# ada-shen/Interpret_quality

Measured on AMD Instinct MI355X. Metric: coalitions/sec (masked forward passes/sec), PointNet 1024-pt ModelNet10, higher is better.
Workload: dtype f32; 1 GPU; PointNet ModelNet10-style Shapley, 32 regions x 1000 permutations per cloud (33000 coalitions per step per GPU), BASELINE configs[1]; permutations sampled and masked on the device inside the timed step; num_points=1024, num_regions=32, permutations=1000, parallelism=clouds sharded over 1 GPU(s), one all_gather_into_tensor of the logits per step

## Files before the change

interpret_quality_amd/csrc/iq_api.hip:

```cpp
#include <algorithm>
#include <vector>

#include "../../include/iq_debug.h"
#include "iq_common.h"
#include "iq_profile.h"

extern "C" int iq_version(void) { return IQ_ABI_VERSION; }

extern "C" const char* iq_last_error(void) { return iq::err_buf(); }

namespace iq {
namespace {
struct Span { hipEvent_t start, stop; int which; double work; };
struct ThreadState {
    std::vector<Span> spans;
    bool enabled = false;
    bool no_lds_gemm = false;
    int twin = 0;
};
ThreadState& ts() {
    static thread_local ThreadState s;
    return s;
}
}

bool profile_enabled() { return ts().enabled; }

bool no_lds_gemm() { return ts().no_lds_gemm; }
int twin() { return ts().twin; }

ProfileSpan::ProfileSpan(int which, hipStream_t st, double work) : which_(which), st_(st), on_(ts().enabled), work_(work) {
    if (!on_) return;
    (void)hipEventCreate(&start_);
    (void)hipEventCreate(&stop_);
    (void)hipEventRecord(start_, st_);
}

ProfileSpan::~ProfileSpan() {
    if (!on_) return;
    (void)hipEventRecord(stop_, st_);
    ts().spans.push_back(Span{start_, stop_, which_, work_});
}
}

extern "C" int iq_set_tuning(int key, int value) {
    if (key == iq::kTuneNoLdsGemm && (value == 0 || value == 1)) {
        iq::ts().no_lds_gemm = value != 0;
        return IQ_OK;
    }
    if (key == iq::kTuneTwin) {
        switch (value) {
            case 0: case iq::kTwinEdgeGemmL2: case iq::kTwinEdgeGemmLds: case iq::kTwinKnnCompact: case iq::kTwinPcKnn:
            case iq::kTwinPcGroupedMlp: case iq::kTwinKnnFp32Rank: case iq::kTwinPn2MemberWalk: case iq::kTwinKnnFp32Mfma:
            case iq::kTwinPcTwoKernel: case iq::kTwinChainL3Fp32: case iq::kTwinChainL3Fp32NoTail16: case iq::kTwinGroupFp32:
            case iq::kTwinDenseFp32: case iq::kTwinChainL3Single: case iq::kTwinDenseTile128: case iq::kTwinGroupFp32Chunk64:
                iq::ts().twin = value;
                return IQ_OK;
        }
    }
    return iq::fail(IQ_EINVAL, "iq_set_tuning: key %d value %d is not an experiment knob", key, value);
}

extern "C" int iq_profile_enable(int on) {
    iq::ts().enabled = on != 0;
    return IQ_OK;
}

extern "C" int iq_profile_read_work(int which, double* total_ms, int* launches, double* total_work) {
    IQ_REQUIRE(total_ms && launches, "iq_profile_read: null output");
    double tot = 0.0, work = 0.0;
    int n = 0;
    std::vector<iq::Span> rest;
    for (const iq::Span& s : iq::ts().spans) {
        if (s.which != which) { rest.push_back(s); continue; }
        float ms = 0.f;
        if (hipEventSynchronize(s.stop) != hipSuccess || hipEventElapsedTime(&ms, s.start, s.stop) != hipSuccess)
            return iq::fail(IQ_ELAUNCH, "iq_profile_read: event query failed");
        tot += ms;
        work += s.work;
        ++n;
        (void)hipEventDestroy(s.start);
        (void)hipEventDestroy(s.stop);
    }
    iq::ts().spans.swap(rest);
    *total_ms = tot;
    *launches = n;
    if (total_work) *total_work = work;
    return IQ_OK;
}

extern "C" int iq_profile_read(int which, double* total_ms, int* launches) {
    return iq_profile_read_work(which, total_ms, launches, nullptr);
}

namespace {
typedef float dbg_f32x16 __attribute__((ext_vector_type(16)));
typedef __bf16 dbg_bf16x8 __attribute__((ext_vector_type(8)));
typedef unsigned dbg_u32x4 __attribute__((ext_vector_type(4)));
__device__ unsigned long long g_sustained_clk[2];

__device__ inline dbg_bf16x8 dbg_operand(unsigned seed) {
    dbg_u32x4 v;
    for (int i = 0; i < 4; ++i) {
        seed = seed * 1664525u + 1013904223u;
        const unsigned lo = 0x3f80u | ((seed >> 9) & 0x7fu) | ((seed >> 3) & 0x8000u);
        seed = seed * 1664525u + 1013904223u;
        const unsigned hi = 0x3f80u | ((seed >> 9) & 0x7fu) | ((seed >> 3) & 0x8000u);
        v[i] = lo | (hi << 16);
    }
    return __builtin_bit_cast(dbg_bf16x8, v);
}

__global__ __launch_bounds__(256) void mfma_sustained_kernel(float* out, int iters, int seed0) {
    const dbg_bf16x8 a0 = dbg_operand(seed0 + threadIdx.x * 7 + blockIdx.x), a1 = dbg_operand(seed0 * 3 + threadIdx.x * 11 + blockIdx.x);
    const dbg_bf16x8 b0 = dbg_operand(seed0 * 5 + threadIdx.x * 13), b1 = dbg_operand(seed0 * 9 + threadIdx.x * 17);
    unsigned long long t0 = 0, r0 = 0;
    if (threadIdx.x == 0 && blockIdx.x == 0) {
        asm volatile("s_memtime %0\n\ts_waitcnt lgkmcnt(0)" : "=s"(t0)::"memory");
        r0 = __builtin_amdgcn_s_memrealtime();
    }
    dbg_f32x16 c0 = {0}, c1 = {0}, c2 = {0}, c3 = {0};
    for (int it = 0; it < iters; ++it) {
#pragma unroll
        for (int r = 0; r < 4; ++r) {
            c0 = __builtin_amdgcn_mfma_f32_32x32x16_bf16(a0, b0, c0, 0, 0, 0);
            c1 = __builtin_amdgcn_mfma_f32_32x32x16_bf16(a1, b0, c1, 0, 0, 0);
            c2 = __builtin_amdgcn_mfma_f32_32x32x16_bf16(a0, b1, c2, 0, 0, 0);
            c3 = __builtin_amdgcn_mfma_f32_32x32x16_bf16(a1, b1, c3, 0, 0, 0);
        }
    }
    if (threadIdx.x == 0 && blockIdx.x == 0) {
        unsigned long long t1;
        asm volatile("s_memtime %0\n\ts_waitcnt lgkmcnt(0)" : "=s"(t1)::"memory");
        g_sustained_clk[0] = t1 - t0;
        g_sustained_clk[1] = __builtin_amdgcn_s_memrealtime() - r0;
    }
    out[blockIdx.x * blockDim.x + threadIdx.x] = c0[0] + c1[5] + c2[9] + c3[15];
}
// ... 76 lines not shown
```

interpret_quality_amd/csrc/iq_common.h:

```cpp
#pragma once
#include <hip/hip_runtime.h>

#include <cstdarg>
#include <cstdio>

#include "../../include/iq.h"

namespace iq {

inline char* err_buf() {
    static thread_local char buf[512] = {0};
    return buf;
}

inline int fail(int code, const char* fmt, ...) {
    va_list ap;
    va_start(ap, fmt);
    vsnprintf(err_buf(), 512, fmt, ap);
    va_end(ap);
    return code;
}

inline int check_launch(const char* what) {
    hipError_t e = hipGetLastError();
    if (e != hipSuccess) return fail(IQ_ELAUNCH, "%s: %s", what, hipGetErrorString(e));
    return IQ_OK;
}

inline hipStream_t as_stream(iq_stream_t s) { return reinterpret_cast<hipStream_t>(s); }

inline size_t align_up(size_t x, size_t a) { return (x + a - 1) / a * a; }

__host__ __device__ inline bool keep_bit(unsigned long long keep, int rid) {
    return (unsigned)rid < 64u && ((keep >> rid) & 1ull);
}

constexpr int kMaxKeepWords = IQ_MAX_WIDE_REGIONS / 64;

__host__ __device__ inline int keep_words(int R) { return (R + 63) >> 6; }

__device__ __forceinline__ bool keep_bit_wide(const uint64_t* keep, int rid, int R) {
    return (unsigned)rid < (unsigned)R && ((keep[rid >> 6] >> (rid & 63)) & 1ull);
}

template <bool WIDE>
struct WaveKeep {
    unsigned long long k = 0;
    const uint64_t* row = nullptr;
    int R = 64;
    __device__ __forceinline__ WaveKeep(const uint64_t* keep, int b, int R_, int W, int lane, uint64_t* strip) {
        if constexpr (WIDE) {
            if (lane < W) strip[lane] = keep[(size_t)b * W + lane];
            __builtin_amdgcn_fence(__ATOMIC_RELEASE, "wavefront");
            __builtin_amdgcn_wave_barrier();
            __builtin_amdgcn_fence(__ATOMIC_ACQUIRE, "wavefront");
            row = strip;
            R = R_;
        } else {
            k = keep[b];
        }
    }
    __device__ __forceinline__ bool operator()(int rid) const {
        if constexpr (WIDE) return keep_bit_wide(row, rid, R);
        else return keep_bit(k, rid);
    }
};

__device__ inline int xcd_cloud(int block, int wgs_per_cloud, int B) {
    const int c = ((block >> 3) / wgs_per_cloud) * 8 + (block & 7);
    return (c | 3) < B ? (c & ~3) | ((c + (c >> 3)) & 3) : c;
}

}

#define IQ_REQUIRE(cond, ...) \
    do {                      \
        if (!(cond)) return iq::fail(IQ_EINVAL, __VA_ARGS__); \
    } while (0)
```

interpret_quality_amd/csrc/iq_pointnet.hip:

```cpp
#include <algorithm>
#include <type_traits>

#include "iq_common.h"
#include "iq_profile.h"

#include "iq_bf3.h"
#include "iq_mfma.h"

namespace {

constexpr int kFeat = IQ_NUM_FEAT;
constexpr int kMC = 64;
constexpr int kMC96 = 96;
constexpr int kMaxN = 4096;
constexpr int kThreads = 256;
constexpr int kRowCap = kMaxN + kMC;

enum ChainMode { kPrepool = 0, kFstn = 1, kTrunk = 2, kFstn64 = 3, kTrunk64 = 4 };

constexpr int kLd1 = 64 + 4;
constexpr int kLd2 = 128 + 4;

struct ChainArgs {
    const float* clouds;
    int ps, cs, cl;
    const float* centers;
    const uint16_t* rows;
    const int32_t* nrows;
    const int32_t* item_order;
    const int32_t* cloud_of;
    const float* trans;
    const float* w_in;
    const float* w1;
    const float* b1;
    const float* w2;
    const float* b2;
    const float* w3;
    const float* b3;
    const unsigned short* w3_bf3;
    const unsigned short* w2_bf3;
    float* out;
    int32_t* argrow;
    int N, R, items, nclouds, with_centre;
    int tail16;
    int l3_single;
};

struct BRing {
    f32x4 r[8];
};

__device__ __forceinline__ void bring_init(BRing& ring, const WBuf& w3, int wave_s) {
#pragma unroll
    for (int i = 0; i < 8; ++i) ring.r[i] = wbuf_load(w3, (wave_s * 16 + i) * kFragBytes);
}

template <int MTS, bool ARGMAX = false>
__device__ __forceinline__ void l3_pass_v2(const WBuf& w3, const float* abase, int wave_s, float (&runmax)[8], BRing& ring,
                                           int (&runarg)[8], int rowbase = 0, int fh = 0) {
    const int w0 = wave_s * 16 * kFragBytes;
    int wq = w0;
#pragma unroll 1
    for (int q = 0; q < 8; ++q) {
        const int wn = (q < 7) ? wq + 4 * 16 * kFragBytes : w0;
        f32x16 acc0 = {0}, acc1 = {0};
        f32x4 a0n = lds_frag<kLd2>(abase, 0, 0), a1n = a0n;
        if (MTS == 2) a1n = lds_frag<kLd2>(abase, 1, 0);
#pragma unroll
        for (int kb = 0; kb < 16; ++kb) {
            const f32x4 a0 = a0n, a1 = a1n;
            if (kb + 1 < 16) {
                a0n = lds_frag<kLd2>(abase, 0, kb + 1);
                if (MTS == 2) a1n = lds_frag<kLd2>(abase, 1, kb + 1);
            }
            const f32x4 bk = ring.r[kb & 7];
            acc0 = mfma4(a0, bk, acc0);
            if (MTS == 2) acc1 = mfma4(a1, bk, acc1);
            ring.r[kb & 7] = wbuf_load(w3, kb < 8 ? wq + (kb + 8) * kFragBytes : wn + (kb - 8) * kFragBytes);
            if (kb + 1 < 16) __builtin_amdgcn_sched_group_barrier(0x100, MTS, 0);
            __builtin_amdgcn_sched_group_barrier(0x008, 4 * MTS, 0);
            __builtin_amdgcn_sched_group_barrier(0x020, 1, 0);
            __builtin_amdgcn_sched_barrier(0);
        }
        if (ARGMAX) {
            float m = -INFINITY;
            int r = 0;
#pragma unroll
            for (int i = 0; i < 16; ++i) {
                if (acc0[i] > m) { m = acc0[i]; r = rowbase + c_row_i(i) + 4 * fh; }
            }
            if (MTS == 2) {
#pragma unroll
                for (int i = 0; i < 16; ++i)
                    if (acc1[i] > m) { m = acc1[i]; r = rowbase + 32 + c_row_i(i) + 4 * fh; }
            }
#pragma unroll
            for (int i = 0; i < 8; ++i) {
                const bool better = (i == q) && m > runmax[i];
                runarg[i] = better ? r : runarg[i];
                runmax[i] = better ? m : runmax[i];
            }
        } else {
            float m = max16(acc0);
            if (MTS == 2) m = fmaxf(m, max16(acc1));
#pragma unroll
            for (int i = 0; i < 8; ++i) runmax[i] = (i == q) ? fmaxf(runmax[i], m) : runmax[i];
        }
        wq = wn;
    }
}

constexpr int kLdB = 256;
constexpr int kPlaneB = kMC * kLdB;
struct B3Ring { B3 r[4]; };
constexpr int kLd1B = 128;
constexpr int kPlane1B = kMC * kLd1B;

__device__ __forceinline__ B3 b3_load16_l2(const __amdgpu_buffer_rsrc_t& rs, int voff, int nt, int t, int hf) {
    return b3_load_at(rs, voff, (nt * 4 + 2 * t) * 1024 + 256 * hf, 16 * 1024);
}

__device__ __forceinline__ B3 b3_load16(const __amdgpu_buffer_rsrc_t& rs, int voff, int q, int t, int hf, int wave_s) {
    return b3_load_at(rs, voff, (((q & 7) * 4 + wave_s) * 8 + 2 * t) * 1024 + 256 * hf, 32 * 8 * 1024);
}

// ... 123 lines not shown
    for (int d = 0; d < 4; ++d) {
        ring.r[2 * d] = __builtin_bit_cast(f32x4, __builtin_amdgcn_raw_buffer_load_b128(w3.rsrc, voff0, w0 + d * kFragBytes, 0));
        ring.r[2 * d + 1] = __builtin_bit_cast(f32x4, __builtin_amdgcn_raw_buffer_load_b128(w3.rsrc, voff1, w0 + d * kFragBytes, 0));
    }
    int wq = w0;
#pragma unroll 1
    for (int q = 0; q < 8; ++q) {
        const int wn = (q < 7) ? wq + 4 * 16 * kFragBytes : w0;
        f32x4 c0 = {0.f, 0.f, 0.f, 0.f}, c1 = c0;
#pragma unroll
        for (int kb = 0; kb < 16; ++kb) {
            const f32x4 b0 = ring.r[2 * (kb & 3)], b1 = ring.r[2 * (kb & 3) + 1];
            c0 = __builtin_amdgcn_mfma_f32_16x16x4f32(a0[kb], odd ? b0[1] : b0[0], c0, 0, 0, 0);
            c1 = __builtin_amdgcn_mfma_f32_16x16x4f32(a0[kb], odd ? b1[1] : b1[0], c1, 0, 0, 0);
            c0 = __builtin_amdgcn_mfma_f32_16x16x4f32(a1[kb], odd ? b0[3] : b0[2], c0, 0, 0, 0);
            c1 = __builtin_amdgcn_mfma_f32_16x16x4f32(a1[kb], odd ? b1[3] : b1[2], c1, 0, 0, 0);
            const int soff = kb < 12 ? wq + (kb + 4) * kFragBytes : wn + (kb - 12) * kFragBytes;
            ring.r[2 * (kb & 3)] = __builtin_bit_cast(f32x4, __builtin_amdgcn_raw_buffer_load_b128(w3.rsrc, voff0, soff, 0));
            ring.r[2 * (kb & 3) + 1] = __builtin_bit_cast(f32x4, __builtin_amdgcn_raw_buffer_load_b128(w3.rsrc, voff1, soff, 0));
        }
        float m0 = fmaxf(fmaxf(c0[0], c0[1]), fmaxf(c0[2], c0[3])), m1 = fmaxf(fmaxf(c1[0], c1[1]), fmaxf(c1[2], c1[3]));
        m0 = fmaxf(m0, __shfl_xor(m0, 16)); m1 = fmaxf(m1, __shfl_xor(m1, 16));
        m0 = fmaxf(m0, __shfl_xor(m0, 32)); m1 = fmaxf(m1, __shfl_xor(m1, 32));
        const float m = (lane & 16) ? m1 : m0;
#pragma unroll
        for (int i = 0; i < 8; ++i) runmax[i] = (i == q) ? fmaxf(runmax[i], m) : runmax[i];
        wq = wn;
    }
}

template <int ROWS, int PLANEB>
__device__ __forceinline__ void stage0b_planes(unsigned char* act0, const float* xs, const f32x4 (&wi)[4], int t) {
    const int cq = t & 15;
#pragma unroll
    for (int i = 0; i < ROWS / 16; ++i) {
        const int row = (t >> 4) + 16 * i;
        const f32x4 xv = *reinterpret_cast<const f32x4*>(xs + row * 4);
        f32x4 v;
#pragma unroll
        for (int j = 0; j < 4; ++j) v[j] = fmaxf(fmaf(wi[j][2], xv[2], fmaf(wi[j][1], xv[1], wi[j][0] * xv[0])) + wi[j][3], 0.f);
        row4_to_planes<PLANEB>(act0 + row * kLd1B + 16 * ((cq >> 1) ^ swz_of_row<kLd1B>(row)) + 8 * (cq & 1), v);
    }
}

struct L1Raw { f32x4 r[2][2]; };
__device__ __forceinline__ L1Raw l1_raw_load(const __amdgpu_buffer_rsrc_t& rs, int ln, int wave_s) {
    const int voff = ((ln >> 4) * 64 + 16 * (wave_s & 1) + (ln & 15)) * 16;
    L1Raw w;
#pragma unroll
    for (int t = 0; t < 2; ++t)
#pragma unroll
        for (int h = 0; h < 2; ++h)
            w.r[t][h] = __builtin_bit_cast(f32x4, __builtin_amdgcn_raw_buffer_load_b128(rs, voff + 512 * h, ((wave_s >> 1) * 8 + 4 * t) * kFragBytes, 0));
    return w;
}
template <int MT, int PLANEB, bool RELU>
__device__ __forceinline__ void l1_bf3(const unsigned char* act0, unsigned char* act1, const L1Raw& raw, f32x4 bq, int ln, int wave_s) {
    constexpr int G = MT % 3 == 0 ? 3 : 2;
    static_assert(MT % G == 0, "m-tiles go G at a time");
    const int a0off = a16_lane_off<kLd1B>(ln), l15 = ln & 15;
    const B3 w[2] = {b3_split8(raw.r[0][0], raw.r[0][1]), b3_split8(raw.r[1][0], raw.r[1][1])};
#pragma unroll
    for (int p = 0; p < MT; p += G) {
        f32x4 acc[G];
#pragma unroll
        for (int i = 0; i < G; ++i) acc[i] = (f32x4){0.f, 0.f, 0.f, 0.f};
#pragma unroll
        for (int t = 0; t < 2; ++t) {
            bf16x8 af[G][3];
#pragma unroll
            for (int i = 0; i < G; ++i) a16_load<kLd1B, PLANEB>(af[i], act0, a0off, p + i, t);
            mfma16_bf3_col_tr<G>(w[t], af, acc);
        }
#pragma unroll
        for (int i = 0; i < G; ++i) {
            f32x4 v = acc[i];
            if (RELU) v = (f32x4){fmaxf(v[0] + bq[0], 0.f), fmaxf(v[1] + bq[1], 0.f), fmaxf(v[2] + bq[2], 0.f), fmaxf(v[3] + bq[3], 0.f)};
            c16_tile_to_planes_swz<kLd1B, PLANEB>(act1, 16 * (p + i) + l15, 2 * wave_s, ln, v);
        }
        __builtin_amdgcn_sched_barrier(0);
    }
}

template <int CM, int L3V, bool ARGMAX = false>
__global__ __launch_bounds__(kThreads, L3V == 3 ? 2 : 3) void pn_chain_kernel(ChainArgs a) {
    constexpr int MODE = CM >= kFstn64 ? CM - kFstn64 + kFstn : CM;
    constexpr int MC = (CM == kFstn || CM == kTrunk) && L3V == 3 && !ARGMAX ? kMC96 : kMC;
    static_assert(CM < kFstn64 || (L3V == 3 && !ARGMAX), "kFstn64 / kTrunk64: the 64-row twins of the product instantiations only");
    __shared__ __attribute__((aligned(16))) float bufA[L3V == 3 ? 3 * MC * kLdB / 4 : kMC * kLd2];
    __shared__ __attribute__((aligned(16))) float bufB[MC == kMC96 ? 4 : (L3V == 3 ? 3 * kPlane1B / 4 : kMC * kLd1)];
    __shared__ __attribute__((aligned(16))) float xs[MC * 4];

    const int tid = threadIdx.x, lane = tid & 63, wave = tid >> 6;
    const int item = a.item_order ? a.item_order[blockIdx.x] : blockIdx.x;
    const int N = a.N;
    int cloud;
    if (MODE == kPrepool) cloud = item / (a.R + a.with_centre);
    else cloud = a.cloud_of ? a.cloud_of[item] : (a.nclouds == 1 ? 0 : item);

    const int nrows = a.nrows[item] & 0xffff;
    float* outp = a.out + (size_t)item * kFeat;
    if (nrows == 0) {
        for (int c = tid; c < kFeat; c += kThreads) outp[c] = -INFINITY;
        return;
    }
    const int nchunks = (nrows + MC - 1) / MC;

    const int c0 = tid & 63, rg = tid >> 6;
    const f32x4 win = *reinterpret_cast<const f32x4*>(a.w_in + c0 * 4);
    const int wave_s = uniform(wave);
    const WBuf w1b = wbuf_make((MODE == kTrunk) ? a.w1 + (size_t)item * 4096 : a.w1, lane);
    const WBuf w2b = wbuf_make(a.w2, lane), w3b = wbuf_make(a.w3, lane);
    const int frag_lane = (lane & 31), frag_h = lane >> 5;
    const float* a1base_A = bufA + frag_lane * kLd1 + 4 * frag_h;
    const float* a1base_B = bufB + frag_lane * kLd1 + 4 * frag_h;
    const float* a2base = bufA + frag_lane * kLd2 + 4 * frag_h;
    float* c1base = bufB + (4 * frag_h) * kLd1 + frag_lane;
    float* c2base = bufA + (4 * frag_h) * kLd2 + frag_lane;

    constexpr int NRUN = L3V == 3 ? 16 : 8;
    float runmax[NRUN];
    int runarg[NRUN];
#pragma unroll
    for (int q = 0; q < NRUN; ++q) { runmax[q] = -INFINITY; runarg[q] = 0; }

    const bool fetcher = lane < MC / 4;
    const int frow = wave * (MC / 4) + lane;
    const uint16_t* rowp = a.rows + (size_t)item * kRowCap + frow;
    float px = 0.f, py = 0.f, pz = 0.f;
    auto load_point = [&](int p) {
        if (p == N) {
            px = a.centers[cloud * 3]; py = a.centers[cloud * 3 + 1]; pz = a.centers[cloud * 3 + 2];
        } else {
            const float* src = a.clouds + (size_t)cloud * a.cl + (size_t)p * a.ps;
            px = src[0]; py = src[a.cs]; pz = src[2 * a.cs];
        }
    };
    int pnext = 0;
    if (fetcher) {
        load_point(rowp[0]);
        if (nchunks > 1) pnext = rowp[MC];
    }

    BRing ring;
    if (L3V == 2) bring_init(ring, w3b, wave_s);
    [[maybe_unused]] B3Ring ring3;
    [[maybe_unused]] const __amdgpu_buffer_rsrc_t w3rs =
        __builtin_amdgcn_make_buffer_rsrc(const_cast<unsigned short*>(L3V == 3 ? a.w3_bf3 : nullptr), 0, 0x7fffffff, 0x00020000);
    [[maybe_unused]] const __amdgpu_buffer_rsrc_t w2rs =
        __builtin_amdgcn_make_buffer_rsrc(const_cast<unsigned short*>(L3V == 3 ? a.w2_bf3 : nullptr), 0, 0x7fffffff, 0x00020000);
    if (L3V == 3) {
#pragma unroll
        for (int i = 0; i < 4; ++i) {
            const bool single = MC == kMC;
            ring3.r[i] = b3_load16(w3rs, b16_lane_off(lane), single ? 0 : i >> 1, single ? i >> 1 : 0, i & 1, wave_s);
        }
    }
    if constexpr (MC == kMC96) {
        auto chunk = [&](auto mtc, const int ch) {
            constexpr int mts = decltype(mtc)::value;
            constexpr int kPlane96 = kMC96 * kLdB, kPlane96_1 = kMC96 * kLd1B, kAct1Off = 3 * kPlane96 - 3 * kPlane96_1;
            static_assert(3 * kPlane96_1 <= kAct1Off, "act0 and act1 are disjoint");
            unsigned char* const img = reinterpret_cast<unsigned char*>(bufA);
            unsigned char* const act1 = img + kAct1Off;
            int ln = lane;
            asm volatile("" : "+v"(ln));
            const int l15 = ln & 15, kq = ln >> 4;
            f32x4 wi[4];
#pragma unroll
            for (int j = 0; j < 4; ++j) wi[j] = *reinterpret_cast<const f32x4*>(a.w_in + ((ln & 15) * 4 + j) * 4);
            if (fetcher) {
                float x = px, y = py, z = pz;
                const float* t9 = a.trans + (size_t)item * 9;
                const float x2 = fmaf(z, t9[6], fmaf(y, t9[3], x * t9[0]));
                const float y2 = fmaf(z, t9[7], fmaf(y, t9[4], x * t9[1]));
                const float z2 = fmaf(z, t9[8], fmaf(y, t9[5], x * t9[2]));
                *reinterpret_cast<f32x4*>(xs + frow * 4) = (f32x4){x2, y2, z2, 0.f};
            }
            __syncthreads();
            if (fetcher && ch + 1 < nchunks) {
                load_point(pnext);
                if (ch + 2 < nchunks) pnext = rowp[(ch + 2) * MC];
            }
// ... 571 lines not shown
__global__ __launch_bounds__(kThreads) void pn_order_count_kernel(const int32_t* __restrict__ nrows_all,
                                                                  int32_t* __restrict__ bin_of, int32_t* __restrict__ hist,
                                                                  int B) {
    __shared__ int lh[kBins];
    if (threadIdx.x < kBins) lh[threadIdx.x] = 0;
    __syncthreads();
    const int item = blockIdx.x * blockDim.x + threadIdx.x;
    if (item < B) {
        const int rows = nrows_all[item] & 0xffff;
        const int bin = kBins - 1 - min(kBins - 1, (rows + kMC - 1) / kMC);
        bin_of[item] = bin;
        atomicAdd(&lh[bin], 1);
    }
    __syncthreads();
    if (threadIdx.x < kBins && lh[threadIdx.x]) atomicAdd(&hist[threadIdx.x], lh[threadIdx.x]);
}

__global__ void pn_order_scan_kernel(int32_t* __restrict__ hist) {
    if (threadIdx.x == 0) {
        int run = 0;
        for (int b = 0; b < kBins; ++b) { const int c = hist[b]; hist[b] = run; run += c; }
    }
}

__global__ __launch_bounds__(kThreads) void pn_order_scatter_kernel(const int32_t* __restrict__ bin_of,
                                                                    int32_t* __restrict__ cursor,
                                                                    int32_t* __restrict__ order, int B) {
    __shared__ int lh[kBins], base[kBins];
    if (threadIdx.x < kBins) lh[threadIdx.x] = 0;
    __syncthreads();
    const int item = blockIdx.x * blockDim.x + threadIdx.x;
    int bin = 0, pos = 0;
    if (item < B) {
        bin = bin_of[item];
        pos = atomicAdd(&lh[bin], 1);
    }
    __syncthreads();
    if (threadIdx.x < kBins && lh[threadIdx.x]) base[threadIdx.x] = atomicAdd(&cursor[threadIdx.x], lh[threadIdx.x]);
    __syncthreads();
    if (item < B) order[base[bin] + pos] = item;
}

constexpr int kOrderThreads = 1024, kOrderPer = 4, kOrderFusedMax = kOrderThreads * kOrderPer;

__global__ __launch_bounds__(kOrderThreads) void pn_order_fused_kernel(const int32_t* __restrict__ nrows_all,
                                                                       int32_t* __restrict__ order, int B) {
    __shared__ int lh[kBins];
    const int tid = threadIdx.x, lane = tid & 63;
    if (tid < kBins) lh[tid] = 0;
    __syncthreads();
    int bin[kOrderPer], pos[kOrderPer];
#pragma unroll
    for (int j = 0; j < kOrderPer; ++j) {
        const int item = tid + j * kOrderThreads;
        if (item < B) {
            const int rows = nrows_all[item] & 0xffff;
            bin[j] = kBins - 1 - min(kBins - 1, (rows + kMC - 1) / kMC);
            pos[j] = atomicAdd(&lh[bin[j]], 1);
        }
    }
    __syncthreads();
    if (tid < 64) {
        int carry = 0;
        for (int b0 = 0; b0 < kBins; b0 += 64) {
            const int b = b0 + lane, c = b < kBins ? lh[b] : 0;
            int inc = c;
#pragma unroll
            for (int off = 1; off < 64; off <<= 1) {
                const int t = __shfl_up(inc, off);
                if (lane >= off) inc += t;
            }
            if (b < kBins) lh[b] = carry + inc - c;
            carry += __shfl(inc, 63);
        }
    }
    __syncthreads();
#pragma unroll
    for (int j = 0; j < kOrderPer; ++j) {
        const int item = tid + j * kOrderThreads;
        if (item < B) order[lh[bin[j]] + pos[j]] = item;
    }
}

__global__ __launch_bounds__(kThreads) void pn_stn_gather_kernel(const float* __restrict__ G,
                                                                 const int32_t* __restrict__ nrows_all,
                                                                 const uint64_t* __restrict__ keep,
                                                                 const int32_t* __restrict__ cloud_of,
                                                                 float* __restrict__ out, int R, int nclouds,
                                                                 int with_centre) {
    const int item = blockIdx.x;
    const int cloud = cloud_of ? cloud_of[item] : (nclouds == 1 ? 0 : item);
    const uint64_t full = R >= 64 ? ~0ull : ((1ull << R) - 1);
    const uint64_t k = (keep ? keep[item] : ~0ull) & full;
    const int per = R + with_centre;
    const f32x4* g4 = reinterpret_cast<const f32x4*>(G) + (size_t)cloud * per * (kFeat / 4) + threadIdx.x;
    f32x4 m = {-INFINITY, -INFINITY, -INFINITY, -INFINITY};
    for (int r = 0; r < R; ++r) {
        if ((k >> r) & 1) {
            const f32x4 v = g4[(size_t)r * (kFeat / 4)];
            m[0] = fmaxf(m[0], v[0]); m[1] = fmaxf(m[1], v[1]); m[2] = fmaxf(m[2], v[2]); m[3] = fmaxf(m[3], v[3]);
        }
    }
    if (nrows_all[item] >> 16) {
        const f32x4 v = g4[(size_t)R * (kFeat / 4)];
        m[0] = fmaxf(m[0], v[0]); m[1] = fmaxf(m[1], v[1]); m[2] = fmaxf(m[2], v[2]); m[3] = fmaxf(m[3], v[3]);
    }
    reinterpret_cast<f32x4*>(out)[(size_t)item * (kFeat / 4) + threadIdx.x] = m;
}

__global__ __launch_bounds__(kThreads) void pn_stn_gather_wide_kernel(const float* __restrict__ G,
                                                                      const int32_t* __restrict__ nrows_all,
                                                                      const uint64_t* __restrict__ keep,
                                                                      const int32_t* __restrict__ cloud_of,
                                                                      float* __restrict__ out, int R, int W, int nclouds,
                                                                      int with_centre) {
    __shared__ uint64_t ks[kMaxW];
    const int item = blockIdx.x;
    const int cloud = cloud_of ? cloud_of[item] : (nclouds == 1 ? 0 : item);
    if ((int)threadIdx.x < W) {
        uint64_t k = keep ? keep[(size_t)item * W + threadIdx.x] : ~0ull;
        if ((int)threadIdx.x == W - 1 && (R & 63)) k &= (1ull << (R & 63)) - 1;
        ks[threadIdx.x] = k;
    }
    __syncthreads();
    const int per = R + with_centre;
    const f32x4* g4 = reinterpret_cast<const f32x4*>(G) + (size_t)cloud * per * (kFeat / 4) + threadIdx.x;
    f32x4 m = {-INFINITY, -INFINITY, -INFINITY, -INFINITY};
    for (int w = 0; w < W; ++w) {
        const uint64_t kw = ks[w];
        uint64_t k = ((uint64_t)(unsigned)__builtin_amdgcn_readfirstlane((int)(kw >> 32)) << 32) |
                     (unsigned)__builtin_amdgcn_readfirstlane((int)kw);
        while (k) {
            int r[4];
#pragma unroll
            for (int q = 0; q < 4; ++q) {
                r[q] = k ? w * 64 + __ffsll((long long)k) - 1 : r[0];
                k &= k - 1;
            }
            f32x4 v[4];
#pragma unroll
            for (int q = 0; q < 4; ++q) v[q] = g4[(size_t)r[q] * (kFeat / 4)];
#pragma unroll
            for (int q = 0; q < 4; ++q) {
                m[0] = fmaxf(m[0], v[q][0]); m[1] = fmaxf(m[1], v[q][1]); m[2] = fmaxf(m[2], v[q][2]); m[3] = fmaxf(m[3], v[q][3]);
            }
        }
    }
    if (nrows_all[item] >> 16) {
        const f32x4 v = g4[(size_t)R * (kFeat / 4)];
        m[0] = fmaxf(m[0], v[0]); m[1] = fmaxf(m[1], v[1]); m[2] = fmaxf(m[2], v[2]); m[3] = fmaxf(m[3], v[3]);
    }
    reinterpret_cast<f32x4*>(out)[(size_t)item * (kFeat / 4) + threadIdx.x] = m;
}

constexpr int kPrefixRows = 8;

__global__ __launch_bounds__(64) void pn_stn_prefix_kernel(const float* __restrict__ G, const int32_t* __restrict__ nrows_all,
                                                           const int32_t* __restrict__ orders,
                                                           const int32_t* __restrict__ cloud_of, float* __restrict__ out,
                                                           int32_t* __restrict__ item_cloud, int R, int nclouds, int with_centre) {
    __shared__ int first_s[IQ_MAX_WIDE_REGIONS];
    __shared__ int src_s[IQ_MAX_WIDE_REGIONS];
    __shared__ unsigned char flag_s[IQ_MAX_WIDE_REGIONS + 1];
    const int o = blockIdx.x, part = blockIdx.y, lane = threadIdx.x;
    const int cloud = cloud_of ? cloud_of[o] : (nclouds == 1 ? 0 : o);
    const int32_t* ord = orders + (size_t)o * R;
// ... 19 lines not shown
            const int r = __builtin_amdgcn_readfirstlane(i < R ? src_s[i] : -1);
            v[q] = r >= 0 ? g4[(size_t)r * (kFeat / 4)] : ninf;
        }
#pragma unroll
        for (int q = 0; q < kPrefixRows; ++q) {
            const int i = i0 + q;
            if (i > R) break;
            f32x4 w = m;
            if (flag_s[i]) { w[0] = fmaxf(w[0], c[0]); w[1] = fmaxf(w[1], c[1]); w[2] = fmaxf(w[2], c[2]); w[3] = fmaxf(w[3], c[3]); }
            o4[(size_t)i * (kFeat / 4)] = w;
            m[0] = fmaxf(m[0], v[q][0]); m[1] = fmaxf(m[1], v[q][1]); m[2] = fmaxf(m[2], v[q][2]); m[3] = fmaxf(m[3], v[q][3]);
        }
    }
}

__global__ __launch_bounds__(kThreads) void pn_fill_rows_kernel(float* __restrict__ out, const float* __restrict__ image, int B) {
    const size_t t = (size_t)blockIdx.x * kThreads + threadIdx.x;
    if (t >= (size_t)B * 1024) return;
    reinterpret_cast<f32x4*>(out)[t] = reinterpret_cast<const f32x4*>(image)[t & 1023];
}

template <int MODE>
void launch_chain(const ChainArgs& a, hipStream_t st) {
    const bool fp32_l3 = iq::twin() == iq::kTwinChainL3Fp32 || iq::twin() == iq::kTwinChainL3Fp32NoTail16;
    const bool bf3 = a.w3_bf3 && a.w2_bf3 && !fp32_l3;
    if constexpr (MODE == kTrunk) {
        if (a.argrow) {
            if (bf3) hipLaunchKernelGGL((pn_chain_kernel<kTrunk, 3, true>), dim3(a.items), dim3(kThreads), 0, st, a);
            else     hipLaunchKernelGGL((pn_chain_kernel<kTrunk, 2, true>), dim3(a.items), dim3(kThreads), 0, st, a);
            return;
        }
    }
    if constexpr (MODE != kPrepool) {
        if (bf3) {
            if (a.l3_single) hipLaunchKernelGGL((pn_chain_kernel<MODE - kFstn + kFstn64, 3>), dim3(a.items), dim3(kThreads), 0, st, a);
            else             hipLaunchKernelGGL((pn_chain_kernel<MODE, 3>), dim3(a.items), dim3(kThreads), 0, st, a);
            return;
        }
    }
    hipLaunchKernelGGL((pn_chain_kernel<MODE, 2>), dim3(a.items), dim3(kThreads), 0, st, a);
}

}

namespace {
using iq::launch_linear;

struct Workspace {
    uint16_t* sorted_pts;
    int32_t* roff;
    uint16_t* rows_pre;
    int32_t* nrows_pre;
    uint16_t* rows;
    int32_t* nrows;
    int32_t* order;
    int32_t* bin_of;
    int32_t* hist;
    float* G;
    float* gbuf;
    float* h1;
    float* h2;
    float* trans;
    float* tfp;
    uint16_t* fc3_bf3;
    size_t bytes;
};

Workspace carve(void* base, int B, int nclouds, int N, int R, int roff_entries = IQ_MAX_REGIONS + 1) {
    Workspace w;
    size_t off = 0;
    auto take = [&](size_t bytes) {
        size_t o = off;
        off = iq::align_up(off + bytes, 256);
        return reinterpret_cast<char*>(base) + o;
    };
    w.sorted_pts = reinterpret_cast<uint16_t*>(take((size_t)nclouds * N * sizeof(uint16_t)));
    w.roff = reinterpret_cast<int32_t*>(take((size_t)nclouds * roff_entries * sizeof(int32_t)));
    w.rows_pre = reinterpret_cast<uint16_t*>(take((size_t)nclouds * (R + 1) * kRowCap * sizeof(uint16_t)));
    w.nrows_pre = reinterpret_cast<int32_t*>(take((size_t)nclouds * (R + 1) * sizeof(int32_t)));
    w.rows = reinterpret_cast<uint16_t*>(take((size_t)B * kRowCap * sizeof(uint16_t)));
    w.nrows = reinterpret_cast<int32_t*>(take((size_t)B * sizeof(int32_t)));
    w.order = reinterpret_cast<int32_t*>(take((size_t)B * sizeof(int32_t)));
    w.bin_of = reinterpret_cast<int32_t*>(take((size_t)B * sizeof(int32_t)));
    w.hist = reinterpret_cast<int32_t*>(take((size_t)kBins * sizeof(int32_t)));
    w.G = reinterpret_cast<float*>(take((size_t)nclouds * (R + 1) * kFeat * sizeof(float)));
    w.gbuf = reinterpret_cast<float*>(take((size_t)B * kFeat * sizeof(float)));
    w.h1 = reinterpret_cast<float*>(take((size_t)B * 512 * sizeof(float)));
    w.h2 = reinterpret_cast<float*>(take((size_t)B * 256 * sizeof(float)));
    w.trans = reinterpret_cast<float*>(take((size_t)B * 9 * sizeof(float)));
    w.tfp = reinterpret_cast<float*>(take((size_t)B * 4096 * sizeof(float)));
    w.fc3_bf3 = reinterpret_cast<uint16_t*>(take(iq_packed_bf3_elems(4096, 256) * sizeof(uint16_t)));
    w.bytes = off;
    return w;
}

}

extern "C" size_t iq_pointnet_workspace_bytes(int B, int nclouds, int N, int R) {
    if (B < 0 || nclouds < 0 || N < 0 || R < 0) return 0;
    return carve(nullptr, B, nclouds, N, R).bytes;
}

extern "C" double iq_pointnet_flops_per_coalition(int N) {
    const double per_point = 426377.0;
    const double fc = 3.0 * (1024.0 * 512 + 512.0 * 256) + 256.0 * (9 + 4096 + 10);
    return 2.0 * (per_point * N + fc);
}

extern "C" int iq_pointnet_coalitions(const iq_pointnet_weights* w, const float* clouds, const float* centers,
                                      const int32_t* region_id, const uint64_t* keep, const int32_t* cloud_of,
                                      float* logits, float* trans_feat_packed, void* workspace,
                                      size_t workspace_bytes, int B, int nclouds, int N, int R,
                                      int channel_first, iq_stream_t stream) {
    return iq_pointnet_coalitions_crt(w, clouds, centers, region_id, keep, cloud_of, logits, trans_feat_packed, nullptr, workspace,
                                      workspace_bytes, B, nclouds, N, R, channel_first, stream);
}

namespace {

int pointnet_coalitions(const iq_pointnet_weights* w, const float* clouds, const float* centers, const int32_t* region_id,
                        const uint64_t* keep, int wide_words, const int32_t* orders, const int32_t* cloud_of, float* logits,
                        float* trans_feat_packed, int32_t* crt_points, void* workspace, size_t workspace_bytes, int B, int nclouds,
                        int N, int R, int channel_first, iq_stream_t stream) {
    const char* who = orders ? "iq_pointnet_prefix_coalitions_wide"
                             : wide_words ? "iq_pointnet_coalitions_wide" : "iq_pointnet_coalitions";
    IQ_REQUIRE(B >= 0 && nclouds >= 1, "%s: B=%d nclouds=%d", who, B, nclouds);
    IQ_REQUIRE(w && clouds && region_id && (logits || B == 0), "%s: null pointer", who);
    IQ_REQUIRE(N >= 1 && N <= kMaxN, "%s: N=%d not in [1,%d]", who, N, kMaxN);
    const int max_regions = wide_words ? IQ_MAX_WIDE_REGIONS : IQ_MAX_REGIONS;
    IQ_REQUIRE(R >= 1 && R <= max_regions, "%s: R=%d not in [1,%d]", who, R, max_regions);
    const int groups = orders ? B / (R + 1) : B;
    IQ_REQUIRE(cloud_of || nclouds == 1 || nclouds == groups, "%s: cloud_of required when 1 < nclouds != %s", who, orders ? "S" : "B");
    const int with_centre = centers ? 1 : 0;
    IQ_REQUIRE(centers || !(keep || orders), "%s: %s need centers", who, orders ? "prefix coalitions" : "keep masks");
    if (B == 0) return IQ_OK;
    const size_t need = wide_words ? iq_pointnet_wide_workspace_bytes(B, nclouds, N, R) : iq_pointnet_workspace_bytes(B, nclouds, N, R);
    if (!workspace || workspace_bytes < need)
        return iq::fail(IQ_EWORKSPACE, "%s: workspace %zu < %zu bytes", who, workspace_bytes, need);
    Workspace ws = wide_words ? carve(workspace, B, nclouds, N, R, R + 1) : carve(workspace, B, nclouds, N, R);
    hipStream_t st = iq::as_stream(stream);
    int rc;
    iq::ProfileSpan call_span(iq::kSlotCall, st);

    const int pre_items = nclouds * (R + with_centre);
    const int32_t* item_cloud = orders ? (nclouds > 1 ? ws.bin_of : nullptr) : cloud_of;
    if (wide_words) {
        hipLaunchKernelGGL(pn_prepare_wide_kernel, dim3(nclouds), dim3(kThreads), 0, st, region_id, ws.sorted_pts, ws.roff, N, R);
        if ((rc = iq::check_launch("pn_prepare_wide_kernel"))) return rc;
        hipLaunchKernelGGL(pn_rows_wide_kernel, dim3(pre_items), dim3(64), 0, st, ws.sorted_pts, ws.roff, nullptr, nullptr,
                           ws.rows_pre, ws.nrows_pre, N, R, wide_words, nclouds, with_centre, 1);
        if ((rc = iq::check_launch("pn_rows_wide_kernel"))) return rc;
        if (orders) {
            hipLaunchKernelGGL(pn_rows_prefix_kernel, dim3(groups), dim3(kThreads), 0, st, ws.sorted_pts, ws.roff, orders, cloud_of,
                               ws.rows, ws.nrows, N, R, nclouds, with_centre);
            if ((rc = iq::check_launch("pn_rows_prefix_kernel"))) return rc;
        } else {
            hipLaunchKernelGGL(pn_rows_wide_kernel, dim3(B), dim3(64), 0, st, ws.sorted_pts, ws.roff, keep, cloud_of, ws.rows,
                               ws.nrows, N, R, wide_words, nclouds, with_centre, 0);
            if ((rc = iq::check_launch("pn_rows_wide_kernel"))) return rc;
        }
    } else {
        hipLaunchKernelGGL(pn_prepare_kernel, dim3(nclouds), dim3(kThreads), 0, st, region_id, ws.sorted_pts, ws.roff, N, R);
        if ((rc = iq::check_launch("pn_prepare_kernel"))) return rc;
        hipLaunchKernelGGL(pn_rows_kernel, dim3(pre_items), dim3(64), 0, st, ws.sorted_pts, ws.roff, nullptr, nullptr,
                           ws.rows_pre, ws.nrows_pre, N, R, nclouds, with_centre, 1);
        hipLaunchKernelGGL(pn_rows_kernel, dim3(B), dim3(64), 0, st, ws.sorted_pts, ws.roff, keep, cloud_of, ws.rows,
                           ws.nrows, N, R, nclouds, with_centre, 0);
        if ((rc = iq::check_launch("pn_rows_kernel"))) return rc;
    }
    if (B <= kOrderFusedMax) {
        hipLaunchKernelGGL(pn_order_fused_kernel, dim3(1), dim3(kOrderThreads), 0, st, ws.nrows, ws.order, B);
    } else {
        if (hipMemsetAsync(ws.hist, 0, kBins * sizeof(int32_t), st) != hipSuccess)
            return iq::fail(IQ_ELAUNCH, "%s: memset failed", who);
        hipLaunchKernelGGL(pn_order_count_kernel, dim3((B + kThreads - 1) / kThreads), dim3(kThreads), 0, st, ws.nrows,
                           ws.bin_of, ws.hist, B);
        hipLaunchKernelGGL(pn_order_scan_kernel, dim3(1), dim3(64), 0, st, ws.hist);
        hipLaunchKernelGGL(pn_order_scatter_kernel, dim3((B + kThreads - 1) / kThreads), dim3(kThreads), 0, st,
                           ws.bin_of, ws.hist, ws.order, B);
    }
    if ((rc = iq::check_launch("pn_order kernels"))) return rc;

    ChainArgs a{};
    a.clouds = clouds;
    if (channel_first) { a.ps = 1; a.cs = N; } else { a.ps = 3; a.cs = 1; }
    a.cl = 3 * N;
    a.centers = centers;
    a.rows = ws.rows_pre;
    a.nrows = ws.nrows_pre;
    a.item_order = nullptr;
    a.N = N; a.R = R; a.nclouds = nclouds; a.with_centre = with_centre;
    a.tail16 = iq::twin() != iq::kTwinChainL3Fp32NoTail16;
    a.l3_single = iq::twin() == iq::kTwinChainL3Single;


    a.cloud_of = nullptr; a.trans = nullptr;
    a.w_in = w->stn_in;
    a.w1 = nullptr; a.b1 = nullptr;
    a.w2 = w->stn_c2.w; a.b2 = w->stn_c2.b;
    a.w3 = w->stn_c3.w; a.b3 = w->stn_c3.b;
    a.out = ws.G;
    a.items = pre_items;
    {
        iq::ProfileSpan span(iq::kSlotPrepool, st);
        launch_chain<kPrepool>(a, st);
    }
    if ((rc = iq::check_launch("pn_chain_kernel<prepool>"))) return rc;

    if (orders)
        hipLaunchKernelGGL(pn_stn_prefix_kernel, dim3(groups, kFeat / 256), dim3(64), 0, st, ws.G, ws.nrows, orders, cloud_of, ws.gbuf,
                           item_cloud ? ws.bin_of : nullptr, R, nclouds, with_centre);
    else if (wide_words)
        hipLaunchKernelGGL(pn_stn_gather_wide_kernel, dim3(B), dim3(kThreads), 0, st, ws.G, ws.nrows, keep, cloud_of, ws.gbuf,
                           R, wide_words, nclouds, with_centre);
    else
        hipLaunchKernelGGL(pn_stn_gather_kernel, dim3(B), dim3(kThreads), 0, st, ws.G, ws.nrows, keep, cloud_of, ws.gbuf,
                           R, nclouds, with_centre);
    if ((rc = iq::check_launch(orders ? "pn_stn_prefix_kernel" : wide_words ? "pn_stn_gather_wide_kernel" : "pn_stn_gather_kernel")))
        return rc;
    if ((rc = launch_linear(ws.gbuf, kFeat, w->stn_fc1, ws.h1, 512, B, 1, st, nullptr, nullptr, 0, true))) return rc;
    if ((rc = launch_linear(ws.h1, 512, w->stn_fc2, ws.h2, 256, B, 1, st, nullptr, nullptr, 0, true))) return rc;
    if ((rc = launch_linear(ws.h2, 256, w->stn_fc3, ws.trans, 9, B, 0, st, nullptr, nullptr, 0, true))) return rc;

    a.cloud_of = item_cloud; a.trans = ws.trans;
    a.rows = ws.rows; a.nrows = ws.nrows;
    a.item_order = ws.order;
    a.w_in = w->feat_in;
    a.items = B;
    a.out = ws.gbuf;
    float* tfp = trans_feat_packed ? trans_feat_packed : ws.tfp;
    if (w->fstn_c1.w) {
        a.w1 = w->fstn_c1.w; a.b1 = w->fstn_c1.b;
        a.w2 = w->fstn_c2.w; a.b2 = w->fstn_c2.b;
        a.w3 = w->fstn_c3.w; a.b3 = w->fstn_c3.b; a.w3_bf3 = reinterpret_cast<const unsigned short*>(w->fstn_c3_bf3);
        a.w2_bf3 = reinterpret_cast<const unsigned short*>(w->fstn_c2_bf3);
        {
            iq::ProfileSpan span(iq::kSlotFstn, st);
            launch_chain<kFstn>(a, st);
        }
        if ((rc = iq::check_launch("pn_chain_kernel<fstn>"))) return rc;
        if ((rc = launch_linear(ws.gbuf, kFeat, w->fstn_fc1, ws.h1, 512, B, 1, st, nullptr, nullptr, 0, true))) return rc;
        if ((rc = launch_linear(ws.h1, 512, w->fstn_fc2, ws.h2, 256, B, 1, st, nullptr, nullptr, 0, true))) return rc;
        iq_dense_layer fc3 = w->fstn_fc3;
        IQ_REQUIRE(fc3.cin == 256 && fc3.cout == 4096, "%s: fstn_fc3 is %d -> %d, not 256 -> 4096", who, fc3.cin, fc3.cout);
        if (!fc3.w_bf3 && iq::twin() != iq::kTwinDenseFp32) {
            if ((rc = iq::launch_split_bf3(fc3.w, ws.fc3_bf3, 4096, 256, st))) return rc;
            fc3.w_bf3 = ws.fc3_bf3;
        }
        if ((rc = launch_linear(ws.h2, 256, fc3, tfp, 4096, B, 0, st, nullptr, nullptr, 0, true))) return rc;
    } else {
        IQ_REQUIRE(w->fstn_fc3.b, "%s: without a feature STN, fstn_fc3.b must hold the packed identity", who);
        hipLaunchKernelGGL(pn_fill_rows_kernel, dim3((unsigned)(((size_t)B * 1024 + kThreads - 1) / kThreads)), dim3(kThreads), 0, st,
                           tfp, w->fstn_fc3.b, B);
        if ((rc = iq::check_launch("pn_fill_rows_kernel"))) return rc;
    }

    a.argrow = crt_points;
    a.w1 = tfp; a.b1 = nullptr;
    a.w2 = w->feat_c2.w; a.b2 = w->feat_c2.b;
    a.w3 = w->feat_c3.w; a.b3 = w->feat_c3.b; a.w3_bf3 = reinterpret_cast<const unsigned short*>(w->feat_c3_bf3);
    a.w2_bf3 = reinterpret_cast<const unsigned short*>(w->feat_c2_bf3);
    {
        iq::ProfileSpan span(iq::kSlotTrunk, st);
        launch_chain<kTrunk>(a, st);
    }
    if ((rc = iq::check_launch("pn_chain_kernel<trunk>"))) return rc;
    if ((rc = launch_linear(ws.gbuf, kFeat, w->cls_fc1, ws.h1, 512, B, 1, st, nullptr, nullptr, 0, true))) return rc;
    if ((rc = launch_linear(ws.h1, 512, w->cls_fc2, ws.h2, 256, B, 1, st, nullptr, nullptr, 0, true))) return rc;
    if ((rc = launch_linear(ws.h2, 256, w->cls_fc3, logits, w->cls_fc3.cout, B, 0, st, nullptr, nullptr, 0, true))) return rc;
    return IQ_OK;
}

}

extern "C" int iq_pointnet_coalitions_crt(const iq_pointnet_weights* w, const float* clouds, const float* centers,
                                          const int32_t* region_id, const uint64_t* keep, const int32_t* cloud_of,
                                          float* logits, float* trans_feat_packed, int32_t* crt_points, void* workspace,
                                          size_t workspace_bytes, int B, int nclouds, int N, int R,
                                          int channel_first, iq_stream_t stream) {
    return pointnet_coalitions(w, clouds, centers, region_id, keep, 0, nullptr, cloud_of, logits, trans_feat_packed, crt_points, workspace,
                               workspace_bytes, B, nclouds, N, R, channel_first, stream);
}

extern "C" size_t iq_pointnet_wide_workspace_bytes(int B, int nclouds, int N, int R) {
    if (B < 0 || nclouds < 0 || N < 0 || R < 0) return 0;
    return carve(nullptr, B, nclouds, N, R, R + 1).bytes;
}

extern "C" int iq_pointnet_coalitions_wide(const iq_pointnet_weights* w, const float* clouds, const float* centers,
                                           const int32_t* region_id, const uint64_t* keep, const int32_t* cloud_of,
                                           float* logits, float* trans_feat_packed, void* workspace, size_t workspace_bytes,
                                           int B, int nclouds, int N, int R, int channel_first, iq_stream_t stream) {
    IQ_REQUIRE(R >= 1 && R <= IQ_MAX_WIDE_REGIONS, "iq_pointnet_coalitions_wide: R=%d not in [1,%d]", R, IQ_MAX_WIDE_REGIONS);
    return pointnet_coalitions(w, clouds, centers, region_id, keep, (R + 63) / 64, nullptr, cloud_of, logits, trans_feat_packed,
                               nullptr, workspace, workspace_bytes, B, nclouds, N, R, channel_first, stream);
}

extern "C" int iq_pointnet_prefix_coalitions_wide(const iq_pointnet_weights* w, const float* clouds, const float* centers,
                                                  const int32_t* region_id, const int32_t* orders, const int32_t* cloud_of,
                                                  float* logits, float* trans_feat_packed, void* workspace, size_t workspace_bytes,
                                                  int S, int nclouds, int N, int R, iq_stream_t stream) {
    IQ_REQUIRE(R >= 1 && R <= IQ_MAX_WIDE_REGIONS, "iq_pointnet_prefix_coalitions_wide: R=%d not in [1,%d]", R, IQ_MAX_WIDE_REGIONS);
    IQ_REQUIRE(S >= 0 && S <= 0x7fffffff / (R + 1), "iq_pointnet_prefix_coalitions_wide: S=%d (R=%d)", S, R);
    IQ_REQUIRE(centers && (orders || S == 0), "iq_pointnet_prefix_coalitions_wide: null pointer");
    return pointnet_coalitions(w, clouds, centers, region_id, nullptr, (R + 63) / 64, orders, cloud_of, logits, trans_feat_packed,
                               nullptr, workspace, workspace_bytes, S * (R + 1), nclouds, N, R, 0, stream);
}

extern "C" int iq_pack_fstn_fc3(const float* w, const float* b, float* out_w, float* out_b, int32_t* perm) {
    IQ_REQUIRE(w && b && out_w && out_b, "iq_pack_fstn_fc3: null pointer");
    float* tmp = new float[4096 * 256];
    for (int nt = 0; nt < 2; ++nt)
        for (int kb = 0; kb < 8; ++kb)
            for (int lane = 0; lane < 64; ++lane)
                for (int j = 0; j < 4; ++j) {
                    const int n = nt * 32 + (lane & 31), k = 8 * kb + 4 * (lane >> 5) + j;
                    const int e = ((nt * 8 + kb) * 64 + lane) * 4 + j;
                    const int src = k * 64 + n;
                    for (int c = 0; c < 256; ++c) tmp[(size_t)e * 256 + c] = w[(size_t)src * 256 + c];
                    out_b[e] = b[src] + (k == n ? 1.f : 0.f);
                    if (perm) perm[e] = src;
                }
    const int rc = iq_pack_weight(tmp, out_w, 4096, 256);
    delete[] tmp;
    return rc;
}
```

interpret_quality_amd/csrc/iq_profile.h:

```cpp
#pragma once
#include <hip/hip_runtime.h>

namespace iq {

enum ProfileSlot { kSlotPrepool = 0, kSlotFstn = 1, kSlotTrunk = 2, kSlotCall = 3, kSlotMask = 4, kSlotDominant = 5 };

bool profile_enabled();

enum TuneKey { kTuneNoLdsGemm = 3, kTuneTwin = 5 };
enum Twin {
    kTwinEdgeGemmL2 = 7,
    kTwinEdgeGemmLds = 8,
    kTwinKnnCompact = 12,
    kTwinPcKnn = 14,
    kTwinPcGroupedMlp = 15,
    kTwinKnnFp32Rank = 20,
    kTwinPn2MemberWalk = 21,
    kTwinKnnFp32Mfma = 22,
    kTwinPcTwoKernel = 31,
    kTwinChainL3Fp32 = 54,
    kTwinChainL3Fp32NoTail16 = 55,
    kTwinGroupFp32 = 56,
    kTwinDenseFp32 = 57,
    kTwinChainL3Single = 58,
    kTwinDenseTile128 = 59,
    kTwinGroupFp32Chunk64 = 64,
};
bool no_lds_gemm();
int twin();

class ProfileSpan {
  public:
    ProfileSpan(int which, hipStream_t st, double work = 0.0);
    ~ProfileSpan();
    ProfileSpan(const ProfileSpan&) = delete;
    ProfileSpan& operator=(const ProfileSpan&) = delete;

  private:
    int which_;
    hipStream_t st_;
    bool on_;
    double work_;
    hipEvent_t start_{}, stop_{};
};

}
```

Baseline: 955,600 coalitions/s.

## Skip duplicate full and singleton coalitions in PointNet chain kernels

When all coalitions come from a single cloud, a small kernel finds one representative item for each of two duplicated coalition kinds: the full point set, and a fixed single-row encoding. Every other item of those kinds returns early in the feature-STN and trunk chain kernels. A copy kernel then broadcasts the representative's pooled features and argmax rows to those items. This removes redundant per-permutation work on the largest coalition, at the cost of two extra launches per stage plus a tiny reduction kernel.

```diff
diff --git a/interpret_quality_amd/csrc/iq_api.hip b/interpret_quality_amd/csrc/iq_api.hip
--- a/interpret_quality_amd/csrc/iq_api.hip
+++ b/interpret_quality_amd/csrc/iq_api.hip
@@ -53,7 +53,8 @@
             case 0: case iq::kTwinEdgeGemmL2: case iq::kTwinEdgeGemmLds: case iq::kTwinKnnCompact: case iq::kTwinPcKnn:
             case iq::kTwinPcGroupedMlp: case iq::kTwinKnnFp32Rank: case iq::kTwinPn2MemberWalk: case iq::kTwinKnnFp32Mfma:
             case iq::kTwinPcTwoKernel: case iq::kTwinChainL3Fp32: case iq::kTwinChainL3Fp32NoTail16: case iq::kTwinGroupFp32:
-            case iq::kTwinDenseFp32: case iq::kTwinChainL3Single: case iq::kTwinDenseTile128: case iq::kTwinGroupFp32Chunk64:
+            case iq::kTwinDenseFp32: case iq::kTwinChainL3Single: case iq::kTwinDenseTile128: case iq::kTwinChainNoDedup:
+            case iq::kTwinGroupFp32Chunk64:
                 iq::ts().twin = value;
                 return IQ_OK;
         }
diff --git a/interpret_quality_amd/csrc/iq_common.h b/interpret_quality_amd/csrc/iq_common.h
--- a/interpret_quality_amd/csrc/iq_common.h
+++ b/interpret_quality_amd/csrc/iq_common.h
@@ -29,7 +29,7 @@
 
 inline hipStream_t as_stream(iq_stream_t s) { return reinterpret_cast<hipStream_t>(s); }
 
-inline size_t align_up(size_t x, size_t a) { return (x + a - 1) / a * a; }
+constexpr size_t align_up(size_t x, size_t a) { return (x + a - 1) / a * a; }
 
 __host__ __device__ inline bool keep_bit(unsigned long long keep, int rid) {
     return (unsigned)rid < 64u && ((keep >> rid) & 1ull);
diff --git a/interpret_quality_amd/csrc/iq_pointnet.hip b/interpret_quality_amd/csrc/iq_pointnet.hip
--- a/interpret_quality_amd/csrc/iq_pointnet.hip
+++ b/interpret_quality_amd/csrc/iq_pointnet.hip
@@ -41,6 +41,7 @@
     const unsigned short* w2_bf3;
     float* out;
     int32_t* argrow;
+    const int32_t* dup_rep;
     int N, R, items, nclouds, with_centre;
     int tail16;
     int l3_single;
@@ -330,6 +331,8 @@
     }
 }
 
+__device__ __forceinline__ int dup_kind(int nrows_word, int N) { return nrows_word == N ? 0 : nrows_word == ((1 << 16) | 1) ? 1 : -1; }
+
 template <int CM, int L3V, bool ARGMAX = false>
 __global__ __launch_bounds__(kThreads, L3V == 3 ? 2 : 3) void pn_chain_kernel(ChainArgs a) {
     constexpr int MODE = CM >= kFstn64 ? CM - kFstn64 + kFstn : CM;
@@ -347,6 +350,10 @@
     else cloud = a.cloud_of ? a.cloud_of[item] : (a.nclouds == 1 ? 0 : item);
 
     const int nrows = a.nrows[item] & 0xffff;
+    if (MODE != kPrepool && a.dup_rep) {
+        const int kind = dup_kind(a.nrows[item], N);
+        if (kind >= 0 && a.dup_rep[kind] != item) return;
+    }
     float* outp = a.out + (size_t)item * kFeat;
     if (nrows == 0) {
         for (int c = tid; c < kFeat; c += kThreads) outp[c] = -INFINITY;
@@ -1084,6 +1091,37 @@
     }
 }
 
+constexpr int kDupRepOff = kBins;
+static_assert(iq::align_up((kBins + 2) * sizeof(int32_t), 256) == iq::align_up(kBins * sizeof(int32_t), 256), "room behind hist");
+
+__global__ __launch_bounds__(kOrderThreads) void pn_dup_rep_kernel(const int32_t* __restrict__ nrows_all, int32_t* __restrict__ rep,
+                                                                   int B, int N) {
+    __shared__ int first[2];
+    if (threadIdx.x < 2) first[threadIdx.x] = B;
+    __syncthreads();
+    for (int item = threadIdx.x; item < B; item += kOrderThreads) {
+        const int kind = dup_kind(nrows_all[item], N);
+        if (kind >= 0) atomicMin(&first[kind], item);
+    }
+    __syncthreads();
+    if (threadIdx.x < 2) rep[threadIdx.x] = first[threadIdx.x];
+}
+
+__global__ __launch_bounds__(kThreads) void pn_dup_copy_kernel(const int32_t* __restrict__ nrows_all, const int32_t* __restrict__ rep,
+                                                               float* __restrict__ out, int32_t* __restrict__ argrow, int N) {
+    const int item = blockIdx.x;
+    const int kind = dup_kind(nrows_all[item], N);
+    if (kind < 0) return;
+    const int src = rep[kind];
+    if (src == item) return;
+    static_assert(kFeat == 4 * kThreads, "one float4 per thread");
+    reinterpret_cast<f32x4*>(out + (size_t)item * kFeat)[threadIdx.x] = reinterpret_cast<const f32x4*>(out + (size_t)src * kFeat)[threadIdx.x];
+    if (argrow) {
+        const int4 v = reinterpret_cast<const int4*>(argrow + (size_t)src * kFeat)[threadIdx.x];
+        reinterpret_cast<int4*>(argrow + (size_t)item * kFeat)[threadIdx.x] = v;
+    }
+}
+
 __global__ __launch_bounds__(kThreads) void pn_stn_gather_kernel(const float* __restrict__ G,
                                                                  const int32_t* __restrict__ nrows_all,
                                                                  const uint64_t* __restrict__ keep,
@@ -1269,7 +1307,7 @@
     w.nrows = reinterpret_cast<int32_t*>(take((size_t)B * sizeof(int32_t)));
     w.order = reinterpret_cast<int32_t*>(take((size_t)B * sizeof(int32_t)));
     w.bin_of = reinterpret_cast<int32_t*>(take((size_t)B * sizeof(int32_t)));
-    w.hist = reinterpret_cast<int32_t*>(take((size_t)kBins * sizeof(int32_t)));
+    w.hist = reinterpret_cast<int32_t*>(take((size_t)(kBins + 2) * sizeof(int32_t)));
     w.G = reinterpret_cast<float*>(take((size_t)nclouds * (R + 1) * kFeat * sizeof(float)));
     w.gbuf = reinterpret_cast<float*>(take((size_t)B * kFeat * sizeof(float)));
     w.h1 = reinterpret_cast<float*>(take((size_t)B * 512 * sizeof(float)));
@@ -1367,6 +1405,12 @@
                            ws.bin_of, ws.hist, ws.order, B);
     }
     if ((rc = iq::check_launch("pn_order kernels"))) return rc;
+    const int32_t* dup_rep = nullptr;
+    if (nclouds == 1 && !wide_words && B > 1 && iq::twin() != iq::kTwinChainNoDedup) {
+        hipLaunchKernelGGL(pn_dup_rep_kernel, dim3(1), dim3(kOrderThreads), 0, st, ws.nrows, ws.hist + kDupRepOff, B, N);
+        if ((rc = iq::check_launch("pn_dup_rep_kernel"))) return rc;
+        dup_rep = ws.hist + kDupRepOff;
+    }
 
     ChainArgs a{};
     a.clouds = clouds;
@@ -1412,6 +1456,7 @@
     a.cloud_of = item_cloud; a.trans = ws.trans;
     a.rows = ws.rows; a.nrows = ws.nrows;
     a.item_order = ws.order;
+    a.dup_rep = dup_rep;
     a.w_in = w->feat_in;
     a.items = B;
     a.out = ws.gbuf;
@@ -1425,6 +1470,7 @@
             iq::ProfileSpan span(iq::kSlotFstn, st);
             launch_chain<kFstn>(a, st);
         }
+        if (dup_rep) hipLaunchKernelGGL(pn_dup_copy_kernel, dim3(B), dim3(kThreads), 0, st, ws.nrows, dup_rep, ws.gbuf, nullptr, N);
         if ((rc = iq::check_launch("pn_chain_kernel<fstn>"))) return rc;
         if ((rc = launch_linear(ws.gbuf, kFeat, w->fstn_fc1, ws.h1, 512, B, 1, st, nullptr, nullptr, 0, true))) return rc;
         if ((rc = launch_linear(ws.h1, 512, w->fstn_fc2, ws.h2, 256, B, 1, st, nullptr, nullptr, 0, true))) return rc;
@@ -1451,6 +1497,7 @@
         iq::ProfileSpan span(iq::kSlotTrunk, st);
         launch_chain<kTrunk>(a, st);
     }
+    if (dup_rep) hipLaunchKernelGGL(pn_dup_copy_kernel, dim3(B), dim3(kThreads), 0, st, ws.nrows, dup_rep, ws.gbuf, crt_points, N);
     if ((rc = iq::check_launch("pn_chain_kernel<trunk>"))) return rc;
     if ((rc = launch_linear(ws.gbuf, kFeat, w->cls_fc1, ws.h1, 512, B, 1, st, nullptr, nullptr, 0, true))) return rc;
     if ((rc = launch_linear(ws.h1, 512, w->cls_fc2, ws.h2, 256, B, 1, st, nullptr, nullptr, 0, true))) return rc;
diff --git a/interpret_quality_amd/csrc/iq_profile.h b/interpret_quality_amd/csrc/iq_profile.h
--- a/interpret_quality_amd/csrc/iq_profile.h
+++ b/interpret_quality_amd/csrc/iq_profile.h
@@ -24,6 +24,7 @@
     kTwinDenseFp32 = 57,
     kTwinChainL3Single = 58,
     kTwinDenseTile128 = 59,
+    kTwinChainNoDedup = 60,
     kTwinGroupFp32Chunk64 = 64,
 };
 bool no_lds_gemm();
```

Result: faster. 1.006 million coalitions/s (median of 6 runs) (+5.3%).
